# Stalfoes/dqn_mgsc_zoo

Hardware: AMD Instinct MI355X
Metric: learner grad-steps/sec at batch=32, 84×84×4 uint8, 1/2/4/8 MI355X (higher is better)
Workload: dtype f32

## Files before the change

dqn_mgsc_zoo_amd/csrc/bwd.hpp:

```cpp
#pragma once
#include "common.hpp"
#include "conv1.hpp"
#include "fwd.hpp"
#include "head.hpp"
#include "sampling.hpp"

namespace dqz {

struct Fc1BwdArgs {
  const float* dz1;
  const float* y3;
  float *th, *mu, *nu;
  int64_t w_off;
  Rms rms;
  int B;
  float* dy3;
  const float *w3, *w2;
  float *w3p, *w2p;
};

__device__ __forceinline__ int w3p_src(int i) {
  const int j = i & 3, kq = (i >> 2) & 3, n = (i >> 4) & 15, w = (i >> 8) & 3, r = i >> 10;
  const int tp = r % 9, nq = r / 9;
  return ((8 - tp) * C3CI + 16 * nq + n) * C3CO + 16 * w + 4 * j + kq;
}
__device__ __forceinline__ int w2p_src(int i) {
  const int j = i & 3, kq = (i >> 2) & 3, n = (i >> 4) & 15, w = (i >> 8) & 3, tp = (i >> 10) & 3;
  const int hh = (i >> 12) & 1, pw = (i >> 13) & 1, ph = (i >> 14) & 1;
  const int kh = ph + 2 * (1 - (tp >> 1)), kw = pw + 2 * (1 - (tp & 1));
  return ((kh * C2K + kw) * C2CI + 16 * hh + n) * C2CO + 16 * w + 4 * j + kq;
}
constexpr int W3P_N = 4 * 9 * 1024, W2P_N = 8 * 4 * 1024;

constexpr int FC1X_LD = 520;

constexpr int FC1X_RED = 256 + 4 * 16;
constexpr int FC1X_SMEM = 32 * FC1X_LD + 4 * 2 * FC1X_RED;

__device__ __forceinline__ void fc1_dx_body(const Fc1BwdArgs& a, float* smem, int blk, int c_beg, int c_end) {
  DQZ_STAMP(5, 0);
  constexpr int LD = FC1X_LD;
  float* s_dz = smem;
  float(*s_red)[2][FC1X_RED] = reinterpret_cast<float(*)[2][FC1X_RED]>(smem + 32 * LD);
  auto red_at = [](int row, int col) { return row * 16 + 16 * (row >> 2) + col; };
  const int t = threadIdx.x, lane = t & 63, w = t >> 6;
  const int n = lane & 15, kq = lane >> 4;
  const int k0 = 16 * blk;
  const float* W1 = a.th + a.w_off;
  float4 wv[8];
#pragma unroll
  for (int j = 0; j < 8; ++j)
    wv[j] = *reinterpret_cast<const float4*>(W1 + (int64_t)(k0 + n) * HID + 128 * w + 16 * j + 4 * kq);
  for (int c = c_beg; c < c_end; c += 32) {
    if (c > c_beg) __syncthreads();
    float4 v[16];
#pragma unroll
    for (int i = 0; i < 16; ++i) {
      const int f = t + 256 * i, row = f >> 7;
      const float4 x = *reinterpret_cast<const float4*>(a.dz1 + (int64_t)min(c + row, a.B - 1) * HID + 4 * (f & 127));
      v[i] = c + row < a.B ? x : make_float4(0.f, 0.f, 0.f, 0.f);
    }
    float ym[2];
#pragma unroll
    for (int h = 0; h < 2; ++h)
      ym[h] = a.y3[(int64_t)min(c + 16 * h + (t >> 4), a.B - 1) * FLAT + k0 + (t & 15)];
#pragma unroll
    for (int i = 0; i < 16; ++i) {
      const int f = t + 256 * i;
      *reinterpret_cast<float4*>(s_dz + (f >> 7) * LD + 4 * (f & 127)) = v[i];
    }
    __syncthreads();
    f32x4 xacc[2] = {f32x4{0.f, 0.f, 0.f, 0.f}, f32x4{0.f, 0.f, 0.f, 0.f}};
#pragma unroll
    for (int mt = 0; mt < 2; ++mt) {
      const float* d = s_dz + (16 * mt + n) * LD + 128 * w + 4 * kq;
#pragma unroll
      for (int j = 0; j < 8; ++j) {
        const float4 av = *reinterpret_cast<const float4*>(d + 16 * j);
        xacc[mt] = mfma4(av.x, wv[j].x, xacc[mt]);
        xacc[mt] = mfma4(av.y, wv[j].y, xacc[mt]);
        xacc[mt] = mfma4(av.z, wv[j].z, xacc[mt]);
        xacc[mt] = mfma4(av.w, wv[j].w, xacc[mt]);
      }
    }
#pragma unroll
    for (int mt = 0; mt < 2; ++mt)
#pragma unroll
      for (int r = 0; r < 4; ++r) s_red[w][mt][red_at(4 * kq + r, n)] = xacc[mt][r];
    __syncthreads();
#pragma unroll
    for (int h = 0; h < 2; ++h) {
      const int sample = c + 16 * h + (t >> 4);
      const int k = red_at(t >> 4, t & 15);
      const float v2 = (s_red[0][h][k] + s_red[1][h][k]) + (s_red[2][h][k] + s_red[3][h][k]);
      if (sample < a.B) a.dy3[(int64_t)sample * FLAT + k0 + (t & 15)] = ym[h] > 0.f ? v2 : 0.f;
    }
  }
  DQZ_STAMP(5, 3);
}

constexpr int C3X_S = 66, C3X_RS = 754, C3X_WIN = 11 * C3X_RS;
constexpr int C3W_S = 80, C3W_RS = 720, C3W_WIN = 9 * C3W_RS;

struct Conv3BwdArgs {
  const float* dy3;
  const float* y2;
  const float* w3;
  const float* w3p;
  float* dy2;
  float* part;
  int B;
  Handoff sync;
};

template <bool PUB>
__device__ __forceinline__ void conv3_bwd_dx(const Conv3BwdArgs& a, float* s_win, int b, int nq, int mh) {
  const int t = threadIdx.x, lane = t & 63, w = t >> 6;
  const int n = lane & 15, kq = lane >> 4;
  float wr[36];
  {
    const float4* wp = reinterpret_cast<const float4*>(a.w3p) + ((nq * 9 * 4 + w) * 16 + n) * 4 + kq;
#pragma unroll
    for (int tp = 0; tp < 9; ++tp) {
      const float4 v = wp[tp * 256];
      wr[4 * tp] = v.x;
      wr[4 * tp + 1] = v.y;
      wr[4 * tp + 2] = v.z;
      wr[4 * tp + 3] = v.w;
    }
  }
  const int ep = min(48 * mh + (t >> 2), C2M - 1);
  const float4 ym4 = *reinterpret_cast<const float4*>(a.y2 + ((int64_t)b * C2M + ep) * C2CO + 16 * nq + 4 * (t & 3));
  const float4* src = reinterpret_cast<const float4*>(a.dy3 + (int64_t)b * FLAT);
  constexpr int NW4 = 121 * 16;
  float4 r[8];
#pragma unroll
  for (int q = 0; q < 8; ++q) {
    const int i = min(t + 256 * q, NW4 - 1);
    const int pix = i >> 4, ph = pix / 11 - 2, pw = pix % 11 - 2;
    const bool in = ph >= 0 && ph < C3O && pw >= 0 && pw < C3O;
    const float4 v = src[(in ? ph * C3O + pw : 0) * 16 + (i & 15)];
    r[q] = in ? v : make_float4(0.f, 0.f, 0.f, 0.f);
  }
  __builtin_amdgcn_sched_barrier(0);
#pragma unroll
  for (int q = 0; q < 8; ++q) {
    const int i = t + 256 * q;
    if (i < NW4) {
      const int pix = i >> 4;
      float* d = s_win + (pix / 11) * C3X_RS + (pix % 11) * C3X_S + win64_ch((i & 15) * 4);
      d[0] = r[q].x;
      d[1] = r[q].y;
      d[2] = r[q].z;
      d[3] = r[q].w;
    }
  }
  __syncthreads();
  DQZ_STAMP(6, 1);
  int base[3];
#pragma unroll
  for (int m = 0; m < 3; ++m) {
    const int p = min(48 * mh + 16 * m + n, C2M - 1);
    base[m] = (p / C2O) * C3X_RS + (p % C2O) * C3X_S + win64_ch(16 * w) + kq;
  }
  f32x4 acc[3];
#pragma unroll
  for (int m = 0; m < 3; ++m) acc[m] = f32x4{0.f, 0.f, 0.f, 0.f};
#pragma unroll
  for (int kk = 0; kk < 36; ++kk) {
    const int tp = kk >> 2;
    const int off = (tp / 3) * C3X_RS + (tp % 3) * C3X_S + 4 * (kk & 3);
#pragma unroll
    for (int m = 0; m < 3; ++m) acc[m] = mfma4(s_win[base[m] + off], wr[kk], acc[m]);
  }
  __syncthreads();
  DQZ_STAMP(6, 2);
  float* s_red = s_win;
#pragma unroll
  for (int m = 0; m < 3; ++m)
#pragma unroll
    for (int rr = 0; rr < 4; ++rr) s_red[w * 768 + (16 * m + 4 * kq + rr) * 16 + n] = acc[m][rr];
  __syncthreads();
  if (t < 192 && 48 * mh + (t >> 2) < C2M) {
    const int i = 4 * t;
    f32x4 v;
#pragma unroll
    for (int e = 0; e < 4; ++e)
      v[e] = (s_red[i + e] + s_red[768 + i + e]) + (s_red[1536 + i + e] + s_red[2304 + i + e]);
    v[0] = ym4.x > 0.f ? v[0] : 0.f;
    v[1] = ym4.y > 0.f ? v[1] : 0.f;
    v[2] = ym4.z > 0.f ? v[2] : 0.f;
    v[3] = ym4.w > 0.f ? v[3] : 0.f;
    float* slab = a.dy2 + (int64_t)b * C2M * C2CO;
    const int off = ((48 * mh + (t >> 2)) * C2CO + 16 * nq + 4 * (t & 3)) * 4;
    if constexpr (PUB)
      store_sc1_f4(slab, C2M * C2CO * 4, off, v);
    else
      *reinterpret_cast<f32x4*>(reinterpret_cast<char*>(slab) + off) = v;
  }
  if constexpr (PUB) a.sync.arrive(b);
}

__device__ __forceinline__ void conv3_bwd_dw(const Conv3BwdArgs& a, float* s_win, int b, int nq) {
  const int t = threadIdx.x, lane = t & 63, w = t >> 6;
  const int n = lane & 15, kq = lane >> 4;
  constexpr int NQ4 = C2M * C2CO / 4;
  float dr[13];
#pragma unroll
  for (int kk = 0; kk < 13; ++kk) {
    const int p = 4 * kk + kq;
    const float v = a.dy3[((int64_t)b * C3M + min(p, C3M - 1)) * C3CO + 16 * nq + n];
    dr[kk] = p < C3M ? v : 0.f;
  }
  float4 r[6];
  {
    const float4* src = reinterpret_cast<const float4*>(a.y2 + (int64_t)b * (C2M * C2CO));
#pragma unroll
    for (int q = 0; q < 6; ++q) r[q] = src[min(t + 256 * q, NQ4 - 1)];
  }
  int pb[13];
#pragma unroll
  for (int kk = 0; kk < 13; ++kk) {
    const int p = min(4 * kk + kq, C3M - 1);
    pb[kk] = (p / C3O) * C3W_RS + (p % C3O) * C3W_S + 16 * w + n;
  }
  f32x4 acc[9];
#pragma unroll
  for (int tp = 0; tp < 9; ++tp) acc[tp] = f32x4{0.f, 0.f, 0.f, 0.f};
#pragma unroll
  for (int q = 0; q < 6; ++q) {
    const int i = t + 256 * q;
    if (i < NQ4) {
      const int pix = i >> 4;
      *reinterpret_cast<float4*>(s_win + (pix / C2O) * C3W_RS + (pix % C2O) * C3W_S + (i & 15) * 4) = r[q];
    }
  }
  __syncthreads();
  DQZ_STAMP(12, 1);
#pragma unroll
  for (int kk = 0; kk < 13; ++kk)
#pragma unroll
    for (int tp = 0; tp < 9; ++tp) {
      const int off = (tp / 3) * C3W_RS + (tp % 3) * C3W_S;
      acc[tp] = mfma4(dr[kk], s_win[pb[kk] + off], acc[tp]);
    }
  float sb = 0.f;
#pragma unroll
  for (int kk = 0; kk < 13; ++kk) sb += dr[kk];
  float* slab = a.part + (int64_t)b * (C3KK + 1) * C3CO;
#pragma unroll
  for (int tp = 0; tp < 9; ++tp)
    *reinterpret_cast<f32x4*>(slab + (tp * C3CI + 16 * w + n) * C3CO + 16 * nq + 4 * kq) = acc[tp];
  if (w == 0) {
    sb += __shfl_xor(sb, 16, 64);
    sb += __shfl_xor(sb, 32, 64);
    if (kq == 0) slab[C3KK * C3CO + 16 * nq + n] = sb;
  }
}

constexpr int C2X_S = 66, C2X_RS = 756, C2X_WIN = 11 * C2X_RS;
constexpr int C2W_S = 40, C2W_RS = 808, C2W_WIN = 20 * C2W_RS;

struct Conv2BwdArgs {
  const float* dy2;
  const float* y1;
  const float* w2;
  const float* w2p;
  float* dy1;
  float* part;
  int B;
  Handoff sync;
  Handoff sync1;
};

struct Conv2DxOps {
  float wr[16];
  float4 ym4[2];
};

__device__ __forceinline__ void conv2_dx_issue(const Conv2BwdArgs& a, int b, int ph, int pw, int hh, float (&wr)[16],
                                               float4 (&ym4)[2]) {
  const int t = threadIdx.x, lane = t & 63, w = t >> 6;
  const int n = lane & 15, kq = lane >> 4;
  {
    const float4* wp =
        reinterpret_cast<const float4*>(a.w2p) + (((((ph * 2 + pw) * 2 + hh) * 4) * 4 + w) * 16 + n) * 4 + kq;
#pragma unroll
    for (int tp = 0; tp < 4; ++tp) {
      const float4 v = wp[tp * 256];
      wr[4 * tp] = v.x;
      wr[4 * tp + 1] = v.y;
      wr[4 * tp + 2] = v.z;
      wr[4 * tp + 3] = v.w;
    }
  }
#pragma unroll
  for (int k = 0; k < 2; ++k) {
    const int q = min((t >> 2) + 64 * k, 99), ah = q / 10, cw = q % 10;
    ym4[k] = *reinterpret_cast<const float4*>(a.y1 + ((int64_t)b * C1M + (2 * ah + ph) * C1O + 2 * cw + pw) * C1CO +
                                              16 * hh + 4 * (t & 3));
  }
}

template <bool WAIT, bool PUB = false, bool PRE = false>
__device__ __forceinline__ void conv2_bwd_dx(const Conv2BwdArgs& a, float* s_win, int b, int ph, int pw, int hh,
                                             const Conv2DxOps* pre = nullptr) {
  const int t = threadIdx.x, lane = t & 63, w = t >> 6;
  const int n = lane & 15, kq = lane >> 4;
  float wr[16];
  float4 ym4[2];
  if constexpr (PRE) {
#pragma unroll
    for (int k = 0; k < 16; ++k) wr[k] = pre->wr[k];
    ym4[0] = pre->ym4[0];
    ym4[1] = pre->ym4[1];
  } else {
    const float4* wp =
        reinterpret_cast<const float4*>(a.w2p) + (((((ph * 2 + pw) * 2 + hh) * 4) * 4 + w) * 16 + n) * 4 + kq;
#pragma unroll
    for (int tp = 0; tp < 4; ++tp) {
      const float4 v = wp[tp * 256];
      wr[4 * tp] = v.x;
      wr[4 * tp + 1] = v.y;
      wr[4 * tp + 2] = v.z;
      wr[4 * tp + 3] = v.w;
    }
#pragma unroll
    for (int k = 0; k < 2; ++k) {
      const int q = min((t >> 2) + 64 * k, 99), ah = q / 10, cw = q % 10;
      ym4[k] = *reinterpret_cast<const float4*>(a.y1 + ((int64_t)b * C1M + (2 * ah + ph) * C1O + 2 * cw + pw) * C1CO +
                                                16 * hh + 4 * (t & 3));
    }
  }
  const float4* src = reinterpret_cast<const float4*>(a.dy2 + (int64_t)b * (C2M * C2CO));
  constexpr int NW4 = 121 * 16;
  if constexpr (WAIT) a.sync.wait(b, kTraceDy2);
  float4 r[8];
#pragma unroll
  for (int q = 0; q < 8; ++q) {
    const int i = min(t + 256 * q, NW4 - 1);
    const int pix = i >> 4, oh = pix / 11 - 1, ow = pix % 11 - 1;
    const bool in = oh >= 0 && oh < C2O && ow >= 0 && ow < C2O;
    const int e = (in ? oh * C2O + ow : 0) * 16 + (i & 15);
    float4 v;
    if constexpr (WAIT)
      v = load_sc1_f4(src, C2M * C2CO * 4, e);
    else
      v = src[e];
    r[q] = in ? v : make_float4(0.f, 0.f, 0.f, 0.f);
  }
  __builtin_amdgcn_sched_barrier(0);
  if constexpr (WAIT) DQZ_STAMP(kTraceDy2, 2);
#pragma unroll
  for (int q = 0; q < 8; ++q) {
    const int i = t + 256 * q;
    if (i < NW4) {
      const int pix = i >> 4;
      float* d = s_win + (pix / 11) * C2X_RS + (pix % 11) * C2X_S + win64_ch((i & 15) * 4);
      d[0] = r[q].x;
      d[1] = r[q].y;
      d[2] = r[q].z;
      d[3] = r[q].w;
    }
  }
  __syncthreads();
  int ack = 0;
  if constexpr (WAIT) ack = a.sync.release_issue(b);
  DQZ_STAMP(7, 1);
  constexpr int MT = 6;
  int base[MT];
#pragma unroll
  for (int m = 0; m < MT; ++m) {
    const int p = min(16 * m + n, 99);
    base[m] = (p / 10) * C2X_RS + (p % 10) * C2X_S + win64_ch(16 * w) + kq;
  }
  f32x4 acc[MT];
#pragma unroll
  for (int m = 0; m < MT; ++m) acc[m] = f32x4{0.f, 0.f, 0.f, 0.f};
  float last[4] = {0.f, 0.f, 0.f, 0.f};
#pragma unroll
  for (int kk = 0; kk < 16; ++kk) {
    const int tp = kk >> 2;
    const int off = (tp >> 1) * C2X_RS + (tp & 1) * C2X_S + 4 * (kk & 3);
#pragma unroll
    for (int m = 0; m < MT; ++m) acc[m] = mfma4(s_win[base[m] + off], wr[kk], acc[m]);
    {
#pragma unroll
      for (int e = 0; e < 4; ++e)
        last[e] = __fmaf_rn(s_win[9 * C2X_RS + (6 + e) * C2X_S + win64_ch(16 * w) + kq + off], wr[kk], last[e]);
    }
  }
  {
#pragma unroll
    for (int e = 0; e < 4; ++e) {
      last[e] += __shfl_xor(last[e], 16, 64);
      last[e] += __shfl_xor(last[e], 32, 64);
    }
  }
  if constexpr (WAIT && !PUB) a.sync.release_finish(b, ack, kTraceDy2);
  __syncthreads();
  DQZ_STAMP(7, 2);
  float* s_red = s_win;
#pragma unroll
  for (int m = 0; m < MT; ++m)
#pragma unroll
    for (int rr = 0; rr < 4; ++rr) s_red[w * 1792 + (16 * m + 4 * kq + rr) * 16 + n] = acc[m][rr];
  if (kq == 0) {
#pragma unroll
    for (int e = 0; e < 4; ++e) s_red[w * 1792 + (96 + e) * 16 + n] = last[e];
  }
  __syncthreads();
#pragma unroll
  for (int k = 0; k < 2; ++k) {
    const int q = (t >> 2) + 64 * k;
    if (q < 100) {
      const int i = 16 * q + 4 * (t & 3), ah = q / 10, cw = q % 10;
      f32x4 v;
#pragma unroll
      for (int e = 0; e < 4; ++e)
        v[e] = (s_red[i + e] + s_red[1792 + i + e]) + (s_red[3584 + i + e] + s_red[5376 + i + e]);
      v[0] = ym4[k].x > 0.f ? v[0] : 0.f;
      v[1] = ym4[k].y > 0.f ? v[1] : 0.f;
      v[2] = ym4[k].z > 0.f ? v[2] : 0.f;
      v[3] = ym4[k].w > 0.f ? v[3] : 0.f;
      float* slab = a.dy1 + (int64_t)b * C1M * C1CO;
      const int off = (((2 * ah + ph) * C1O + 2 * cw + pw) * C1CO + 16 * hh + 4 * (t & 3)) * 4;
      if constexpr (PUB)
        store_sc1_f4(slab, C1M * C1CO * 4, off, v);
      else
        *reinterpret_cast<f32x4*>(reinterpret_cast<char*>(slab) + off) = v;
    }
  }
  if constexpr (PUB) a.sync1.arrive(b);
  if constexpr (WAIT && PUB) a.sync.release_finish(b, ack, kTraceDy2);
}

constexpr int C2V_WIN = 9 * C2W_RS;

__device__ __forceinline__ void conv2_bwd_dw_split(const Conv2BwdArgs& a, float* s_win, int b, int kh, int ch) {
  const int t = threadIdx.x, lane = t & 63, w = t >> 6;
  const int n = lane & 15, kq = lane >> 4;
  constexpr int NV4 = 9 * C1O * C1CO / 4;
  float4 r[6];
  {
    const float4* src = reinterpret_cast<const float4*>(a.y1 + (int64_t)b * (C1M * C1CO));
#pragma unroll
    for (int q = 0; q < 6; ++q) {
      const int i = min(t + 256 * q, NV4 - 1);
      const int oh = i / (C1O * 8), rem = i % (C1O * 8);
      r[q] = src[((2 * oh + kh) * C1O) * 8 + rem];
    }
  }
  int pb[21];
#pragma unroll
  for (int kk = 0; kk < 21; ++kk) {
    const int p = min(4 * kk + kq, C2M - 1);
    pb[kk] = (p / C2O) * C2W_RS + (2 * (p % C2O) + w) * C2W_S + n;
  }
  f32x4 acc[2][2];
#pragma unroll
  for (int mt = 0; mt < 2; ++mt)
#pragma unroll
    for (int ct = 0; ct < 2; ++ct) acc[mt][ct] = f32x4{0.f, 0.f, 0.f, 0.f};
#pragma unroll
  for (int q = 0; q < 6; ++q) {
    const int i = t + 256 * q;
    if (i < NV4) {
      const int oh = i / (C1O * 8), rem = i % (C1O * 8), iw = rem >> 3;
      *reinterpret_cast<float4*>(s_win + oh * C2W_RS + iw * C2W_S + (rem & 7) * 4) = r[q];
    }
  }
  a.sync.wait(b, kTraceDy2);
  float dr[21][2];
#pragma unroll
  for (int kk = 0; kk < 21; ++kk) {
    const int p = 4 * kk + kq;
#pragma unroll
    for (int ct = 0; ct < 2; ++ct) {
      const float* gp = a.dy2 + ((int64_t)b * C2M + min(p, C2M - 1)) * C2CO + 32 * ch + 16 * ct + n;
      const float v = __hip_atomic_load(gp, __ATOMIC_RELAXED, __HIP_MEMORY_SCOPE_AGENT);
      dr[kk][ct] = p < C2M ? v : 0.f;
    }
  }
  DQZ_STAMP(kTraceDy2, 2);
  __syncthreads();
  const int ack = a.sync.release_issue(b);
  DQZ_STAMP(13, 1);
#pragma unroll
  for (int kk = 0; kk < 21; ++kk)
#pragma unroll
    for (int mt = 0; mt < 2; ++mt) {
      const float av = s_win[pb[kk] + 16 * mt];
#pragma unroll
      for (int ct = 0; ct < 2; ++ct) acc[mt][ct] = mfma4(dr[kk][ct], av, acc[mt][ct]);
    }
  a.sync.release_finish(b, ack, kTraceDy2);
  float sb[2] = {0.f, 0.f};
#pragma unroll
  for (int ct = 0; ct < 2; ++ct)
#pragma unroll
    for (int kk = 0; kk < 21; ++kk) sb[ct] += dr[kk][ct];
  float* slab = a.part + (int64_t)b * (C2KK + 1) * C2CO;
#pragma unroll
  for (int mt = 0; mt < 2; ++mt)
#pragma unroll
    for (int ct = 0; ct < 2; ++ct)
      *reinterpret_cast<f32x4*>(slab + ((kh * C2K + w) * C2CI + 16 * mt + n) * C2CO + 32 * ch + 16 * ct + 4 * kq) =
          acc[mt][ct];
  if (kh == 0 && w == 0) {
#pragma unroll
    for (int ct = 0; ct < 2; ++ct) {
      float v = sb[ct];
      v += __shfl_xor(v, 16, 64);
      v += __shfl_xor(v, 32, 64);
      if (kq == 0) slab[C2KK * C2CO + 32 * ch + 16 * ct + n] = v;
    }
  }
}

constexpr int FC1W_LD = 144;
constexpr int FC1W_TLD = 36;
constexpr int FC1W_SMEM = 32 * FC1W_LD + 4 * 16 * FC1W_TLD;

__device__ __forceinline__ void fc1_dw_body(const Fc1BwdArgs& a, float* smem, int blk) {
  DQZ_STAMP(11, 0);
  const int t = threadIdx.x, lane = t & 63, w = t >> 6;
  const int n = lane & 15, kq = lane >> 4;
  const int kb = blk >> 2, nq = blk & 3;
  const int k0 = 16 * kb, c0 = 128 * nq;
  const Rms& R = a.rms;
  const bool upd = R.update();
  float4 v[4];
  float yv[8];
  auto load_chunk = [&](int c) {
#pragma unroll
    for (int i = 0; i < 4; ++i) {
      const int f = t + 256 * i, row = f >> 5;
      const float4 x = *reinterpret_cast<const float4*>(a.dz1 + (int64_t)min(c + row, a.B - 1) * HID + c0 + 4 * (f & 31));
      v[i] = c + row < a.B ? x : make_float4(0.f, 0.f, 0.f, 0.f);
    }
#pragma unroll
    for (int kk = 0; kk < 8; ++kk) {
      const int bb = c + 4 * kk + kq;
      const float y = a.y3[(int64_t)min(bb, a.B - 1) * FLAT + k0 + n];
      yv[kk] = bb < a.B ? y : 0.f;
    }
  };
  load_chunk(0);
  const float* pth = R.meta == 2 ? R.J : R.meta == 3 ? R.G2 : a.th;
  const float* pmu = R.meta >= 2 ? R.mu1 : (upd || R.meta == 1) ? a.mu : a.th;
  const float* pnu = R.meta >= 2 ? R.nu1 : (upd || R.meta == 1) ? a.nu : a.th;
  const int64_t e0 = a.w_off + (int64_t)(k0 + (lane >> 3)) * HID + c0 + 32 * w + 4 * (lane & 7);
  float4 o_th[2], o_mu[2], o_nu[2];
#pragma unroll
  for (int h = 0; h < 2; ++h) {
    const int64_t e = e0 + (int64_t)8 * h * HID;
    o_th[h] = *reinterpret_cast<const float4*>(pth + e);
    o_mu[h] = *reinterpret_cast<const float4*>(pmu + e);
    o_nu[h] = *reinterpret_cast<const float4*>(pnu + e);
  }
  f32x4 gacc[2] = {f32x4{0.f, 0.f, 0.f, 0.f}, f32x4{0.f, 0.f, 0.f, 0.f}};
  for (int c = 0;;) {
#pragma unroll
    for (int i = 0; i < 4; ++i) {
      const int f = t + 256 * i;
      *reinterpret_cast<float4*>(smem + (f >> 5) * FC1W_LD + 4 * (f & 31)) = v[i];
    }
    __syncthreads();
    if (c == 0) DQZ_STAMP(11, 1);
#pragma unroll
    for (int kk = 0; kk < 8; ++kk) {
      const float* d = smem + (4 * kk + kq) * FC1W_LD + 32 * w + n;
      gacc[0] = mfma4(yv[kk], d[0], gacc[0]);
      gacc[1] = mfma4(yv[kk], d[16], gacc[1]);
    }
    c += 32;
    if (c >= a.B) break;
    __syncthreads();
    load_chunk(c);
  }
  DQZ_STAMP(11, 2);
  float* tile = smem + 32 * FC1W_LD + w * 16 * FC1W_TLD;
#pragma unroll
  for (int q = 0; q < 2; ++q)
#pragma unroll
    for (int r = 0; r < 4; ++r) tile[(4 * kq + r) * FC1W_TLD + 16 * q + n] = gacc[q][r];
  float sq = 0.f, s1 = 0.f;
  const float clip = R.meta == 3 ? fminf(fmaxf(R.td[0], -R.bound), R.bound) : 0.f;
#pragma unroll
  for (int h = 0; h < 2; ++h) {
    const float4 g = *reinterpret_cast<const float4*>(tile + ((lane >> 3) + 8 * h) * FC1W_TLD + 4 * (lane & 7));
    const int64_t e = e0 + (int64_t)8 * h * HID;
    if (R.meta == 1) {
      float4 t = o_th[h], m = o_mu[h], v = o_nu[h], j;
      j.x = R.meta1(g.x, t.x, m.x, v.x);
      j.y = R.meta1(g.y, t.y, m.y, v.y);
      j.z = R.meta1(g.z, t.z, m.z, v.z);
      j.w = R.meta1(g.w, t.w, m.w, v.w);
      *reinterpret_cast<float4*>(R.thp + e) = t;
      *reinterpret_cast<float4*>(R.mu1 + e) = m;
      *reinterpret_cast<float4*>(R.nu1 + e) = v;
      *reinterpret_cast<float4*>(R.J + e) = j;
      if (R.gout) *reinterpret_cast<float4*>(R.gout + e) = g;
    } else if (R.meta == 2) {
      float4 o;
      o.x = R.meta2(g.x, o_mu[h].x, o_nu[h].x, o_th[h].x, sq);
      o.y = R.meta2(g.y, o_mu[h].y, o_nu[h].y, o_th[h].y, sq);
      o.z = R.meta2(g.z, o_mu[h].z, o_nu[h].z, o_th[h].z, sq);
      o.w = R.meta2(g.w, o_mu[h].w, o_nu[h].w, o_th[h].w, sq);
      *reinterpret_cast<float4*>(R.vout + e) = o;
    } else if (R.meta == 3) {
      float4 m = o_mu[h], v = o_nu[h];
      R.meta3(g.x, o_th[h].x, m.x, v.x, clip, sq, s1);
      R.meta3(g.y, o_th[h].y, m.y, v.y, clip, sq, s1);
      R.meta3(g.z, o_th[h].z, m.z, v.z, clip, sq, s1);
      R.meta3(g.w, o_th[h].w, m.w, v.w, clip, sq, s1);
      *reinterpret_cast<float4*>(R.gout + e) = g;
      *reinterpret_cast<float4*>(R.mu1 + e) = m;
      *reinterpret_cast<float4*>(R.nu1 + e) = v;
    } else if (!upd) {
      float4 o = g;
      if (R.gacc) {
        const float4 prev = *reinterpret_cast<const float4*>(R.gout + e);
        o.x += prev.x;
        o.y += prev.y;
        o.z += prev.z;
        o.w += prev.w;
      }
      *reinterpret_cast<float4*>(R.gout + e) = o;
    } else {
      float4 m = o_mu[h], vv = o_nu[h], th = o_th[h];
      R.step(g.x, th.x, m.x, vv.x);
      R.step(g.y, th.y, m.y, vv.y);
      R.step(g.z, th.z, m.z, vv.z);
      R.step(g.w, th.w, m.w, vv.w);
      *reinterpret_cast<float4*>(a.mu + e) = m;
      *reinterpret_cast<float4*>(a.nu + e) = vv;
      *reinterpret_cast<float4*>(a.th + e) = th;
    }
  }
  if (R.meta >= 2) {
    sq = wave_sum(sq);
    s1 = wave_sum(s1);
    if (lane == 0) {
      tile[0] = sq;
      tile[1] = s1;
    }
    __syncthreads();
    if (threadIdx.x == 0) {
      const float* t0 = smem + 32 * FC1W_LD;
      constexpr int WT = 16 * FC1W_TLD;
      R.sq_part[R.sq_off + blk] = (t0[0] + t0[WT]) + (t0[2 * WT] + t0[3 * WT]);
      if (R.meta == 3) R.s1_part[R.sq_off + blk] = (t0[1] + t0[WT + 1]) + (t0[2 * WT + 1] + t0[3 * WT + 1]);
    }
  }
  DQZ_STAMP(11, 3);
}


constexpr int FC1X_BLOCKS = FLAT / 16;
inline int fc1_dx_blocks(int B) { return FC1X_BLOCKS * ((B + 31) / 32); }
__device__ __forceinline__ void fc1_dx_block(const Fc1BwdArgs& a, float* smem, int blk) {
  const int g = blk * 256 + threadIdx.x;
  float v3 = 0.f, v2 = 0.f;
  if (a.w3p) {
    if (g < W3P_N) v3 = a.w3[w3p_src(g)];
    if (g < W2P_N) v2 = a.w2[w2p_src(g)];
  }
  const int kb = blk % FC1X_BLOCKS, c = 32 * (blk / FC1X_BLOCKS);
  fc1_dx_body(a, smem, kb, c, min(c + 32, a.B));
  if (a.w3p) {
    if (g < W3P_N) a.w3p[g] = v3;
    if (g < W2P_N) a.w2p[g] = v2;
  }
  DQZ_STAMP(5, 3);
}

constexpr int FC1X1_ROWS = 32;
constexpr int FC1X1_BLOCKS = FLAT / FC1X1_ROWS;

template <int AMAX, int SMAX, int ZMAX>
__global__ __launch_bounds__(512) void head_dx1_kernel(HeadArgs h, Fc1BwdArgs a) {
  __shared__ __attribute__((aligned(16))) float s_dz[HID];
  DQZ_STAMP(5, 0);
  const int half = threadIdx.x >> 8, t = threadIdx.x & 255;
  const int row0 = FC1X1_ROWS * blockIdx.x + 16 * half;
  const int r = row0 + (t >> 4), c0 = 32 * (t & 15);
  const float* W1 = a.th + a.w_off;
  float4 wv[8];
#pragma unroll
  for (int j = 0; j < 8; ++j) wv[j] = *reinterpret_cast<const float4*>(W1 + (int64_t)r * HID + c0 + 4 * j);
  const float ym = a.y3[r];
  const int g = (row0 / 16) * 256 + t;
  float v3 = 0.f, v2 = 0.f;
  if (a.w3p) {
    if (g < W3P_N) v3 = a.w3[w3p_src(g)];
    if (g < W2P_N) v2 = a.w2[w2p_src(g)];
  }
  head_body<AMAX, SMAX, ZMAX>(h, 0, blockIdx.x == 0, s_dz);
  __syncthreads();
  DQZ_STAMP(5, 1);
  float d = 0.f;
#pragma unroll
  for (int j = 0; j < 8; ++j) {
    const float4 z = *reinterpret_cast<const float4*>(s_dz + c0 + 4 * j);
    d = __fmaf_rn(wv[j].x, z.x, d);
    d = __fmaf_rn(wv[j].y, z.y, d);
    d = __fmaf_rn(wv[j].z, z.z, d);
    d = __fmaf_rn(wv[j].w, z.w, d);
  }
  d += dpp_f<0xB1>(d);
  d += dpp_f<0x4E>(d);
  d += dpp_f<0x141>(d);
  d += dpp_f<0x140>(d);
  if ((t & 15) == 0) a.dy3[r] = ym > 0.f ? d : 0.f;
  if (a.w3p) {
    if (g < W3P_N) a.w3p[g] = v3;
    if (g < W2P_N) a.w2p[g] = v2;
  }
  DQZ_STAMP(5, 3);
}

#ifdef DQZ_STEP_TU
inline hipError_t launch_head_dx1(const HeadArgs& h, const Fc1BwdArgs& f, hipStream_t st) {
  if (h.S > 7 || h.Z < 1 || h.Z > 3 || h.B != 1) return hipErrorInvalidValue;
  const dim3 grid(FC1X1_BLOCKS), block(512);
  if (h.A <= 8) {
    if (h.Z <= 2)
      hipLaunchKernelGGL((head_dx1_kernel<8, 7, 2>), grid, block, 0, st, h, f);
    else
      hipLaunchKernelGGL((head_dx1_kernel<8, 7, 3>), grid, block, 0, st, h, f);
  } else {
    if (h.Z <= 2)
      hipLaunchKernelGGL((head_dx1_kernel<MAXA, 7, 2>), grid, block, 0, st, h, f);
    else
      hipLaunchKernelGGL((head_dx1_kernel<MAXA, 7, 3>), grid, block, 0, st, h, f);
  }
  return hipGetLastError();
}
#endif

DQZ_STEP_KERNEL __launch_bounds__(256) void fc1_dx_kernel(Fc1BwdArgs a) {
  __shared__ __attribute__((aligned(16))) float smem[FC1X_SMEM];
  fc1_dx_block(a, smem, blockIdx.x);
}

__device__ __forceinline__ void bwd_chain_block(const Conv3BwdArgs& c3, const Conv2BwdArgs& c2, const Conv1DwArgs& c1,
                                                float* smem, int s, int j) {
  const int ph = (j & 3) >> 1, pw = j & 1, hh = j >> 2, rb = j >> 1, ch = j & 1;
  const int slot = c1.src.slots[s];
  DQZ_STAMP(6, 0);
  conv3_bwd_dx<true>(c3, smem, s, j & 3, j >> 2);
  DQZ_STAMP(6, 3);
  DQZ_STAMP(7, 0);
  Conv2DxOps o2;
  conv2_dx_issue(c2, s, ph, pw, hh, o2.wr, o2.ym4);
  const Conv1DwFrames fr = conv1_dw_frame_ids(c1, ch, slot);
  __builtin_amdgcn_sched_barrier(0);
  conv2_bwd_dx<true, true, true>(c2, smem, s, ph, pw, hh, &o2);
  DQZ_STAMP(7, 3);
  __builtin_amdgcn_s_setprio(2);
  DQZ_STAMP(8, 0);
  const uint4 v = conv1_dw_issue(c1, rb, fr);
  __builtin_amdgcn_sched_barrier(0);
  conv1_dw_body<true>(c1, smem, v, rb, ch, s);
}

constexpr int BWD_CHAIN_MAXB = 64;
inline int bwd_bc_blocks(int B, bool wb, bool chain) {
  const int B8 = (B + 7) / 8 * 8;
  return (wb ? 8 : 0) + 8 * B8 + 4 * (FLAT / 16) + 4 * B8 + 8 * B8 + (chain ? 0 : 16 * B8);
}

template <bool WB, bool CHAIN>
__global__ __launch_bounds__(256) __attribute__((amdgpu_waves_per_eu(4, 8))) void bwd_bc_kernel(
    Conv3BwdArgs c3, Fc1BwdArgs f1, Conv2BwdArgs c2, Conv1DwArgs c1, PerWbArgs wb) {
  constexpr int kW = C3X_WIN > FC1W_SMEM ? C3X_WIN : FC1W_SMEM;
  constexpr int kW2 = C2X_WIN > C3W_WIN ? C2X_WIN : C3W_WIN;
  constexpr int kW3 = C2V_WIN > C1H_SMEM ? C2V_WIN : C1H_SMEM;
  constexpr int kWA = kW > kW2 ? kW : kW2;
  constexpr int kSmem = kWA > kW3 ? kWA : kW3;
  static_assert(kSmem * 4 >= PWB_LDS_BYTES, "the write-back's LDS comes out of the backward's buffer");
  __shared__ __attribute__((aligned(16))) float smem[kSmem];
  const int B8 = (c3.B + 7) / 8 * 8;
  constexpr int NF = 4 * (FLAT / 16);
  int i = blockIdx.x;
  if constexpr (WB) {
    if (i < 8) {
      if (i == 0 && threadIdx.x < 64) per_write_back_wave(wb, reinterpret_cast<char*>(smem));
      return;
    }
    i -= 8;
  }
  if (i < 8 * B8) {
    const SampleJob sj = xcd_sample_job_at(i, 8, c3.B);
    if (!sj.valid) return;
    __builtin_amdgcn_s_setprio(3);
    if constexpr (CHAIN) {
      bwd_chain_block(c3, c2, c1, smem, sj.s, sj.job);
    } else {
      DQZ_STAMP(6, 0);
      conv3_bwd_dx<true>(c3, smem, sj.s, sj.job & 3, sj.job >> 2);
      DQZ_STAMP(6, 3);
    }
    return;
  }
  i -= 8 * B8;
  if (i < NF) {
    fc1_dw_body(f1, smem, i);
    return;
  }
  i -= NF;
  if constexpr (!CHAIN) {
    if (i < 8 * B8) {
      const SampleJob sj = xcd_sample_job_at(i, 8, c2.B);
      if (!sj.valid) return;
      __builtin_amdgcn_s_setprio(3);
      DQZ_STAMP(7, 0);
      conv2_bwd_dx<true, true>(c2, smem, sj.s, (sj.job & 3) >> 1, sj.job & 1, sj.job >> 2);
      DQZ_STAMP(7, 3);
      return;
    }
    i -= 8 * B8;
  }
  if (i < 4 * B8) {
    const SampleJob sj = xcd_sample_job_at(i, 4, c3.B);
    if (!sj.valid) return;
    DQZ_STAMP(12, 0);
    conv3_bwd_dw(c3, smem, sj.s, sj.job);
    DQZ_STAMP(12, 3);
    return;
  }
  i -= 4 * B8;
  if constexpr (!CHAIN) {
    if (i < 8 * B8) {
      const SampleJob sj = xcd_sample_job_at(i, 8, c1.B);
      if (!sj.valid) return;
      __builtin_amdgcn_s_setprio(2);
      conv1_dw_half(c1, smem, sj.job >> 1, sj.job & 1, sj.s);
      return;
    }
    i -= 8 * B8;
  }
  const SampleJob sj = xcd_sample_job_at(i, 8, c2.B);
  if (!sj.valid) return;
  DQZ_STAMP(13, 0);
  conv2_bwd_dw_split(c2, smem, sj.s, sj.job >> 1, sj.job & 1);
  DQZ_STAMP(13, 3);
}

}
```

Measured before the change: 16810.

## Vectorize conv2 dW dy2 loads with DPP quad transpose; reorder CHAIN job dispatch

After: 17180, median of 6. 1.02x the previous value.

```diff
diff --git a/dqn_mgsc_zoo_amd/csrc/bwd.hpp b/dqn_mgsc_zoo_amd/csrc/bwd.hpp
--- a/dqn_mgsc_zoo_amd/csrc/bwd.hpp
+++ b/dqn_mgsc_zoo_amd/csrc/bwd.hpp
@@ -437,6 +437,30 @@
 
 constexpr int C2V_WIN = 9 * C2W_RS;
 
+template <int CTRL>
+__device__ __forceinline__ float quad_perm_f(float v) {
+  return __builtin_bit_cast(float, __builtin_amdgcn_update_dpp(0, __builtin_bit_cast(int, v), CTRL, 0xf, 0xf, true));
+}
+
+__device__ __forceinline__ void quad_transpose4(float (&v)[4]) {
+  const bool b0 = threadIdx.x & 1, b1 = threadIdx.x & 2;
+#pragma unroll
+  for (int h = 0; h < 4; h += 2) {
+    const float lo = v[h], hi = v[h + 1];
+    const float plo = quad_perm_f<0xB1>(lo), phi = quad_perm_f<0xB1>(hi);
+    v[h] = b0 ? phi : lo;
+    v[h + 1] = b0 ? hi : plo;
+  }
+#pragma unroll
+  for (int h = 0; h < 2; ++h) {
+    const float lo = v[h], hi = v[h + 2];
+    const float plo = quad_perm_f<0x4E>(lo), phi = quad_perm_f<0x4E>(hi);
+    v[h] = b1 ? phi : lo;
+    v[h + 2] = b1 ? hi : plo;
+  }
+}
+
+template <bool WIDE>
 __device__ __forceinline__ void conv2_bwd_dw_split(const Conv2BwdArgs& a, float* s_win, int b, int kh, int ch) {
   const int t = threadIdx.x, lane = t & 63, w = t >> 6;
   const int n = lane & 15, kq = lane >> 4;
@@ -472,17 +496,50 @@
   }
   a.sync.wait(b, kTraceDy2);
   float dr[21][2];
-#pragma unroll
-  for (int kk = 0; kk < 21; ++kk) {
-    const int p = 4 * kk + kq;
-#pragma unroll
-    for (int ct = 0; ct < 2; ++ct) {
-      const float* gp = a.dy2 + ((int64_t)b * C2M + min(p, C2M - 1)) * C2CO + 32 * ch + 16 * ct + n;
-      const float v = __hip_atomic_load(gp, __ATOMIC_RELAXED, __HIP_MEMORY_SCOPE_AGENT);
-      dr[kk][ct] = p < C2M ? v : 0.f;
-    }
-  }
-  DQZ_STAMP(kTraceDy2, 2);
+  if constexpr (WIDE) {
+    const float4* src = reinterpret_cast<const float4*>(a.dy2 + (int64_t)b * (C2M * C2CO));
+    const int q4 = n >> 2, e = n & 3;
+    float4 ld[6][2];
+#pragma unroll
+    for (int g = 0; g < 6; ++g)
+#pragma unroll
+      for (int ct = 0; ct < 2; ++ct)
+        ld[g][ct] = load_sc1_f4(src, C2M * C2CO * 4,
+                                min(4 * (4 * g + e) + kq, C2M - 1) * (C2CO / 4) + 8 * ch + 4 * ct + q4);
+    __builtin_amdgcn_sched_barrier(0);
+    DQZ_STAMP(kTraceDy2, 2);
+#pragma unroll
+    for (int g = 0; g < 6; ++g)
+#pragma unroll
+      for (int ct = 0; ct < 2; ++ct) {
+        float v[4] = {ld[g][ct].x, ld[g][ct].y, ld[g][ct].z, ld[g][ct].w};
+        if (g == 5) {
+          const bool in = 4 * (4 * g + e) + kq < C2M;
+#pragma unroll
+          for (int j = 0; j < 4; ++j) v[j] = in ? v[j] : 0.f;
+        }
+        quad_transpose4(v);
+#pragma unroll
+        for (int j = 0; j < 4; ++j)
+          if (4 * g + j < 21) {
+            asm volatile("" : "+v"(v[j]));
+            dr[4 * g + j][ct] = v[j];
+          }
+        __builtin_amdgcn_sched_barrier(0);
+      }
+  } else {
+#pragma unroll
+    for (int kk = 0; kk < 21; ++kk) {
+      const int p = 4 * kk + kq;
+#pragma unroll
+      for (int ct = 0; ct < 2; ++ct) {
+        const float* gp = a.dy2 + ((int64_t)b * C2M + min(p, C2M - 1)) * C2CO + 32 * ch + 16 * ct + n;
+        const float v = __hip_atomic_load(gp, __ATOMIC_RELAXED, __HIP_MEMORY_SCOPE_AGENT);
+        dr[kk][ct] = p < C2M ? v : 0.f;
+      }
+    }
+    DQZ_STAMP(kTraceDy2, 2);
+  }
   __syncthreads();
   const int ack = a.sync.release_issue(b);
   DQZ_STAMP(13, 1);
@@ -823,6 +880,23 @@
     }
     i -= 8 * B8;
   }
+  if constexpr (CHAIN) {
+    if (i < 8 * B8) {
+      const SampleJob sj = xcd_sample_job_at(i, 8, c2.B);
+      if (!sj.valid) return;
+      DQZ_STAMP(13, 0);
+      conv2_bwd_dw_split<true>(c2, smem, sj.s, sj.job >> 1, sj.job & 1);
+      DQZ_STAMP(13, 3);
+      return;
+    }
+    i -= 8 * B8;
+    const SampleJob sj = xcd_sample_job_at(i, 4, c3.B);
+    if (!sj.valid) return;
+    DQZ_STAMP(12, 0);
+    conv3_bwd_dw(c3, smem, sj.s, sj.job);
+    DQZ_STAMP(12, 3);
+    return;
+  }
   if (i < 4 * B8) {
     const SampleJob sj = xcd_sample_job_at(i, 4, c3.B);
     if (!sj.valid) return;
@@ -845,7 +919,7 @@
   const SampleJob sj = xcd_sample_job_at(i, 8, c2.B);
   if (!sj.valid) return;
   DQZ_STAMP(13, 0);
-  conv2_bwd_dw_split(c2, smem, sj.s, sj.job >> 1, sj.job & 1);
+  conv2_bwd_dw_split<false>(c2, smem, sj.s, sj.job >> 1, sj.job & 1);
   DQZ_STAMP(13, 3);
 }
 
```
